# Ajay-Wong/seq2seq-attention-asr

Measured on AMD Instinct MI355X. Metric: log-mel frames/sec fwd+bwd, Chorowski TIMIT baseline, higher is better.
Workload: dtype fp32; 1 GPU; BASELINE config 2: timit_chorowski_b32; model=timit/model_chorowski_baseline.lua, global_batch=32, utterances_per_gpu=32, seq_len=128, label_len=40, feat_dim=123, parallelism=dp1, allreduce=none, launch=hipGraph replay

## Files before the change

### seq2seq-attention-asr_amd/csrc/gru_persist.hip

```cpp
#include <algorithm>
#include <cstdlib>

#include "decisions.h"
#include "gru.h"
#include "gru_persist.h"
#include "handoff.h"
#include "skinny.h"

namespace s2s {

namespace {

struct PDir {
  const float* xp;
  long ldxp;
  const float* Wa;
  const float* Wb;
  float* y;
  long ldy;
  float* sv;
  const float* dy;
  long lddy;
  float* dA;
  long ldA;
// ... 79 lines not shown
  float* part;
  unsigned* ticket;
  unsigned long long* stamps;
};

struct PArgs {
  XProj xq;
  int fused;
  PDir d[2];
  int B, L, H, MT, nwg;
  int nmem, nchains;
  int allow_local;
  unsigned* abort_word;
  unsigned* census;
  const int* len;
  char* next_sync;
  size_t next_prep;
  GruPackJobs pack;
  int ring;
  int stream_sweep;
  unsigned long long* stamps;
  unsigned long long* pstamps;
  int prefetch, prefetch_wg;
  unsigned* progress;
  WArgs wg;
};

#ifndef S2S_GRU_DIAG
#define S2S_GRU_DIAG 0
#endif
constexpr int kStampSlots = S2S_GRU_DIAG ? 16 : 8;
#define GRU_STAMP(ph)                                                                      \
  do {                                                                                     \
    if (a.stamps && threadIdx.x == 0)                                                      \
      a.stamps[((long)lw * a.L + s) * kStampSlots + (ph)] = __builtin_amdgcn_s_memrealtime(); \
  } while (0)
#define GRU_STAMP_V(ph, v)                                                                 \
  do {                                                                                     \
    if (a.stamps && threadIdx.x == 0) a.stamps[((long)lw * a.L + s) * kStampSlots + (ph)] = (v); \
  } while (0)
#if S2S_GRU_DIAG
template <int NC>
__device__ __forceinline__ bool sweep_sent_n(float4 (&a)[NC], __amdgpu_buffer_rsrc_t rs, long tbase, int rowt,
                                             int wave, int lane, unsigned* abort_word, unsigned& n) {
  const long lo = tbase + 4 * tile_lane(rowt, lane);
  unsigned spins = 0;
  while (true) {
    ++n;
    bool ok = true;
#pragma unroll
    for (int i = 0; i < NC; ++i) {
      const long off = lo + 4L * 256 * (wave + 4 * i);
      const uint4 p = __builtin_bit_cast(uint4, __builtin_amdgcn_raw_buffer_load_b128(rs, (int)off, 0, 16));
      ok = ok && p.x != kSent && p.y != kSent && p.z != kSent && p.w != kSent;
      a[i] = make_float4(__uint_as_float(p.x), __uint_as_float(p.y), __uint_as_float(p.z), __uint_as_float(p.w));
    }
    if (__all(ok)) return true;
    if (spin_give_up(spins, abort_word)) return false;
  }
}
#define SWEEP_SENT(slot_, ...) sweep_sent_n<NC>(__VA_ARGS__, npoll[slot_])
#else
#define SWEEP_SENT(slot_, ...) sweep_sent_tile<NC>(__VA_ARGS__)
#endif
std::atomic<unsigned long long*> g_gru_stamps[2] = {{nullptr}, {nullptr}};
std::atomic<unsigned long long*> g_gru_pstamps[2] = {{nullptr}, {nullptr}};
std::atomic<unsigned long long*> g_gru_wstamps{nullptr};
constexpr int kProdStampItems = 32;

__device__ __forceinline__ float reduce_or_abort(SkinnyRed& red, int* abort_lds, bool ok, floatx4 acc, int wave,
                                                 int lane, int tid, bool* aborted) {
  if (!ok) *abort_lds = 1;
  const float s = skinny_reduce(red, acc, wave, lane, tid);
  *aborted = *abort_lds != 0;
  return s;
}

template <bool NN, int D>
__device__ __forceinline__ void xproj_produce(const PArgs& a, float* lds, int p, int nprod) {
  const XProj& q = a.xq;
  const int tid = threadIdx.x, lane = tid & 63, wave = tid >> 6;
  const int nk = q.K / 32;
  __shared__ int last_part;
  const int nd = q.nd;
  if (tid >= 256) {
    XUnit x;
    for (int it = 0; xunit_of(q, nd, p, nprod, it, x); ++it) {
      const int nb = 1 + nk / x.P + (q.alpha ? 1 : 0);
      for (int i = 0; i < nb; ++i) __syncthreads();
      if (x.P == 1) {
        __syncthreads();
      } else {
        __syncthreads();
        __syncthreads();
        if (last_part) __syncthreads();
      }
    }
    return;
  }
  const int wy = wave >> 1, wx = wave & 1, li = lane & 31, lk = lane >> 5;
  const int B = a.B, L = a.L, H3 = q.ncd;
  constexpr int LDK = 36;
  float* As[2] = {lds, lds + 64 * LDK};
  float* Bs[2] = {lds + 128 * LDK, lds + 192 * LDK};
  int item = 0;
  XUnit xu;
  for (; xunit_of(q, nd, p, nprod, item, xu); ++item) {
    if (a.pstamps && tid == 0 && item < kProdStampItems)
      a.pstamps[((long)p * kProdStampItems + item) * 2] = __builtin_amdgcn_s_memrealtime();
// ... 210 lines not shown
    const int upto = nr ? ready + (int)__builtin_ctzll(nr) : ready + 64;
    if (upto <= need && spin_give_up(spins, abort_word)) break;
    ready = upto;
  }
}

__device__ __forceinline__ void prep_next_sync(const PArgs& a, int sp, int nsp) {
  if (!a.next_sync) return;
  if (sp == 0 && threadIdx.x == 0) {
    unsigned* hdr = reinterpret_cast<unsigned*>(a.next_sync);
    const unsigned e = __hip_atomic_fetch_add(&g_s2s_epoch_ctr, 1u, __ATOMIC_RELAXED, __HIP_MEMORY_SCOPE_AGENT) + 1u;
    __hip_atomic_exchange(hdr + kEpochWord, e, __ATOMIC_RELAXED, __HIP_MEMORY_SCOPE_AGENT);
    rearm_abort_word(hdr);
  }
  const size_t n16 = (a.next_prep - 256) / 16;
  uint4* p = reinterpret_cast<uint4*>(a.next_sync + 256);
  for (size_t i = (size_t)sp * blockDim.x + threadIdx.x; i < n16; i += (size_t)nsp * blockDim.x)
    p[i] = make_uint4(0u, 0u, 0u, 0u);
  if (threadIdx.x == 0 && sp == 0 && (a.next_prep - 256) % 16) {
    unsigned* t = reinterpret_cast<unsigned*>(a.next_sync + 256 + n16 * 16);
    for (size_t i = 0; i < ((a.next_prep - 256) % 16) / 4; ++i) t[i] = 0u;
  }
}

constexpr int kRowRing = 4;
constexpr int kSentRing = 4;
__device__ __forceinline__ int sent_slot(const PArgs& a, int s) { return a.ring ? (s & (a.ring - 1)) : s; }
__device__ __forceinline__ void rearm_tile(float* role, const PArgs& a, int s, long tile, int lane) {
  const float4 sv = make_float4(__uint_as_float(kSent), __uint_as_float(kSent), __uint_as_float(kSent),
                                __uint_as_float(kSent));
  *reinterpret_cast<float4*>(role + (long)sent_slot(a, s) * a.MT * 16 * a.H + tile + 4 * lane) = sv;
}
constexpr int kFwdThreads = 320;
template <int NC>
__global__ __launch_bounds__(kFwdThreads) void gru_fwd_persist(PArgs a) {
  __shared__ SkinnyRed red;
  __shared__ int abort_lds, local_lds;
  __shared__ unsigned tb_lds;
  __shared__ __attribute__((aligned(16))) float hprev[16][16];
  __shared__ __attribute__((aligned(16))) float xring[kRowRing][2][256];
  __shared__ __attribute__((aligned(16))) float stg[2][3][256];
  extern __shared__ __attribute__((aligned(16))) float xlds[];
  const int H = a.H, B = a.B, L = a.L;
  const ChainSlot cs = chain_slot(a.nmem);
  if (cs.chain >= a.nchains) {
    const int gch = 8 * ((a.nchains + 7) / 8);
    const int sp = (cs.chain - a.nchains) * a.nmem + cs.member, nsp = (gch - a.nchains) * a.nmem;
    prep_next_sync(a, sp, nsp);
    if (a.fused) xproj_produce_any<false>(a, xlds, sp, nsp);
    for (int j = 0; j < a.pack.n; ++j)
      gru_pack_elems(a.pack.j[j], (long)sp * blockDim.x + threadIdx.x, (long)nsp * blockDim.x);
    return;
  }
  const int dir = cs.chain / a.MT, mt = cs.chain % a.MT;
  const PDir& g = a.d[dir];
  const int ncol = 2 * H / 16;
  const int c1 = cs.member;
  const int lw = dir * a.nwg + mt * ncol + c1;
  const bool isz = c1 < H / 16;
  const int tid = threadIdx.x, lane = tid & 63, wave = tid >> 6;
  const int b0 = mt * 16;
  if (tid == 0) abort_lds = 0;
  const unsigned tb = launch_tagbase(a.abort_word, &tb_lds);
  const bool loader = wave == 4;
  const long mytile = (long)mt * 16 * H + (long)(isz ? c1 : c1 - H / 16) * 256;
  if (!loader)
    rearm_rect((isz ? g.s0 : g.s1) + mytile, (long)a.MT * 16 * H, a.ring ? a.ring : L, 16, 0, 16, 0, 16);
// ... 59 lines not shown
      if (s > 0) store(s - 1);
      put(s + 2, ra);
      issue(s + 3, ra);
      if (ring) {
        if (isz && s >= 2) rearm_tile(g.s0, a, s - 2, mytile, lane);
        if (!isz && s >= 1) rearm_tile(g.s1, a, s - 1, mytile, lane);
      }
      if (!isz) continue;
      __syncthreads();
      if (abort_lds) return;
    }
    __syncthreads();
    store(L - 1);
    return;
  }

  float4 w1[NC], w2[NC];
  load_wfrag(w1, g.Wa + (long)(c1 * 16 + (lane & 15)) * H, wave, lane);
  if (isz) load_wfrag(w2, g.Wb + (long)(c1 * 16 + (lane & 15)) * H, wave, lane);

  const __amdgpu_buffer_rsrc_t hg = rsrc_of(g.g0), qg = rsrc_of(g.g1), hs = rsrc_of(g.s0), qs = rsrc_of(g.s1);
  const long slot = (long)B * H;
  const long slotS = (long)a.MT * 16 * H, tileS = (long)mt * 16 * H;
  const int rowt = min(b0 + (lane & 15), B - 1) - b0;
  const int br = min(b0 + (lane & 15), B - 1);
  const int ob = b0 + (tid >> 4), on = c1 * 16 + (tid & 15);
  const bool live = ob < B;
  const int lenb = (a.len && live) ? a.len[ob] : L;
  const int jt = c1 * 16 - H, wt = (jt % 64) / 16, it = jt / 64;
  float zreg = 0.f, hreg = 0.f;
  bool aborted = false;

  __syncthreads();
  for (int s = 0; s < L; ++s) {
    const int t = g.reverse ? L - 1 - s : s;
    floatx4 acc = {0.f, 0.f, 0.f, 0.f};
    bool ok = true;
    GRU_STAMP(0);
    if (s > 0) {
      float4 av[NC];
#if S2S_GRU_DIAG
      unsigned npoll[1] = {0};
#endif
      {
      if (loc) ok = SWEEP_SENT(0, av, hs, 4 * (sent_slot(a, s - 1) * slotS + tileS), rowt, wave, lane, a.abort_word);
      else ok = sweep_skinny<NC>(av, hg, 8 * (((s - 1) & 1) * slot + (long)br * H), tb + s, wave, lane, a.abort_word);
      GRU_STAMP(1);
#if S2S_GRU_DIAG
      GRU_STAMP_V(8, npoll[0]);
#endif
      acc = mfma_chunks<NC>(av, w1);
      }
      if (!isz && wave == wt) {
#pragma unroll
        for (int i = 0; i < NC; ++i)
          if (i == it) *reinterpret_cast<float4*>(&hprev[lane & 15][4 * (lane >> 4)]) = av[i];
      }
    }
    GRU_STAMP(6);
    float sum = reduce_or_abort(red, &abort_lds, ok, acc, wave, lane, tid, &aborted);
    GRU_STAMP(7);
    const float xpv = xring[s % kRowRing][0][tid], xph = xring[s % kRowRing][1][tid];
    const float hpark = hprev[tid >> 4][tid & 15];
    {
      const float gate = gru_sigmoid(sum + xpv);
      float* st3 = &stg[s & 1][0][tid];
      if (isz) {
        st3[0] = gate;
        zreg = gate;
      } else {
        const int j = on - H;
        const float hp = s > 0 ? hpark : 0.f;
        const float q = gate * hp;
        if (loc) {
          if (live) put_sent(g.s1 + sent_slot(a, s) * slotS + tile_off(ob, j, H), q);
        } else {
          put_granule_pair(g.g1, (s & 1) * slot + (long)ob * H + j, q, tb + s + 1, live);
        }
        st3[0] = gate;
        st3[256] = hp;
        st3[512] = q;
      }
    }
    GRU_STAMP(2);
    if (aborted) return;
    if (!isz) continue;
    acc = floatx4{0.f, 0.f, 0.f, 0.f};
    ok = true;
    GRU_STAMP(3);
    if (s > 0) {
      float4 av[NC];
#if S2S_GRU_DIAG
      unsigned npoll[1] = {0};
#endif
      {
      if (loc) ok = SWEEP_SENT(0, av, qs, 4 * (sent_slot(a, s) * slotS + tileS), rowt, wave, lane, a.abort_word);
      else ok = sweep_skinny<NC>(av, qg, 8 * ((s & 1) * slot + (long)br * H), tb + s + 1, wave, lane, a.abort_word);
      GRU_STAMP(4);
#if S2S_GRU_DIAG
      GRU_STAMP_V(9, npoll[0]);
#endif
      acc = mfma_chunks<NC>(av, w2);
      }
    }
    sum = reduce_or_abort(red, &abort_lds, ok, acc, wave, lane, tid, &aborted);
    {
      const float hh = gru_tanh(sum + xph);
      const float hp = hreg;
      hreg = (-zreg + 1.0f) * hp + zreg * hh;
      if (t >= lenb) hreg = 0.f;
      if (loc) {
        if (live) put_sent(g.s0 + sent_slot(a, s) * slotS + tile_off(ob, on, H), hreg);
      } else {
        put_granule_pair(g.g0, (s & 1) * slot + (long)ob * H + on, hreg, tb + s + 1, live);
      }
      stg[s & 1][1][tid] = hh;
      stg[s & 1][2][tid] = hreg;
    }
    GRU_STAMP(5);
    if (aborted) return;
  }
  __syncthreads();
}

constexpr int kBwdThreads = 320;

template <int NC>
__device__ __forceinline__ void bptt_prefetch(const PArgs& a, int chain, int w, int nwg) {
  if (threadIdx.x >= 256) return;
  const int tid = threadIdx.x, L = a.L, H = a.H, B = a.B, nmem = a.nmem;
  const int tasks = 64 * nmem / nwg, task0 = w * tasks;
  const int dir = chain / a.MT, mt = chain % a.MT;
  const PDir& g = a.d[dir];
  const unsigned* prog = a.progress + (long)chain * nmem;
  int yready = 0, have = 0;
  float sink = 0.f;
  __shared__ int have_lds[2];
  int it = 0;
  constexpr int kMaxTasks = NC;
  for (int q = 3; q < L; ++q, ++it) {
    if (tid == 0) {
      unsigned spins = 0;
      bool gave_up = false;
      while (have + 3 + a.prefetch < q) {
        have = (int)__hip_atomic_load(prog, __ATOMIC_RELAXED, __HIP_MEMORY_SCOPE_AGENT);
        if (have + 3 + a.prefetch >= q) break;
        if (spin_give_up(spins, a.abort_word)) {
          gave_up = true;
          break;
        }
      }
      have_lds[it & 1] = gave_up ? -1 : have;
    }
    __syncthreads();
    const int hv = have_lds[it & 1];
    if (hv < 0) return;
    have = hv;
    if (q < have + 4) q = have + 4;
// ... 177 lines not shown
  const __amdgpu_buffer_rsrc_t pr = rsrc_of(q.part);
  const int tile = 3 * H * NP;
  const int mine = (dir * a.MT + mt) * tile + row0 * NP + (4 * kq) * NP + cb0 * 16 + jl;
#pragma unroll
  for (int c = 0; c < kWgCB; ++c) {
    if (cb0 + c >= nblk) continue;
#pragma unroll
    for (int r = 0; r < 4; ++r)
#pragma unroll
      for (int e = 0; e < 4; ++e)
        __builtin_amdgcn_raw_buffer_store_b32(__float_as_uint(acc[r][c][e]), pr, 4 * (mine + (16 * r + e) * NP + 16 * c),
                                              0, 16);
  }
  asm volatile("s_waitcnt vmcnt(0)" ::: "memory");
  __syncthreads();
  if (tid == 0)
    *flag_lds = (int)__hip_atomic_fetch_add(q.ticket + dir * q.nw + w, 1u, __ATOMIC_RELAXED, __HIP_MEMORY_SCOPE_AGENT);
  __syncthreads();
  if (*flag_lds != a.MT - 1) return;
  const long ldw = (long)H + D;
  float* dW = q.dW[dir][gate];
  const int u0 = row0 - gate * H, first = dir * a.MT * tile + row0 * NP;
  for (int idx = tid; idx < 64 * NP; idx += 256) {
    const int rr = idx / NP, j = idx - rr * NP;
    if (j >= H + D) continue;
    float sum = __uint_as_float(__builtin_amdgcn_raw_buffer_load_b32(pr, 4 * (first + idx), 0, 16));
    for (int m = 1; m < a.MT; ++m)
      sum += __uint_as_float(__builtin_amdgcn_raw_buffer_load_b32(pr, 4 * (first + m * tile + idx), 0, 16));
    float* o = dW + (long)(u0 + rr) * ldw + j;
    *o = q.scale * sum + *o;
  }
}

template <int NC>
__global__ __launch_bounds__(kBwdThreads) void gru_bwd_persist(PArgs a) {
  __shared__ SkinnyRed red;
  __shared__ int abort_lds, local_lds;
  __shared__ unsigned tb_lds;
  __shared__ __attribute__((aligned(16))) float rowq[kRowRing][5][256];
  extern __shared__ __attribute__((aligned(16))) float ylds[];
  const int H = a.H, B = a.B, L = a.L;
  const ChainSlot cs = chain_slot(a.nmem);
  const int gch = 8 * ((a.nchains + 7) / 8);
  if ((int)blockIdx.x >= chain_grid(a.nchains, a.nmem)) {
    const int pre = chain_grid(a.nchains, a.nmem) + (a.prefetch ? 8 * a.prefetch_wg : 0);
    if ((int)blockIdx.x < pre) {
      const int e = (int)blockIdx.x - chain_grid(a.nchains, a.nmem), c = e & 7, w = e >> 3;
      if (c < a.nchains) bptt_prefetch<NC>(a, c, w, a.prefetch_wg);
      return;
    }
    const int e = (int)blockIdx.x - pre, c = e & 7, w = e >> 3;
    if (c < a.nchains) bptt_wgrad<NC>(a, c, w, &tb_lds, &abort_lds);
    return;
  }
  if (cs.chain >= a.nchains) {
    const int sp = (cs.chain - a.nchains) * a.nmem + cs.member, nsp = (gch - a.nchains) * a.nmem;
    prep_next_sync(a, sp, nsp);
    if (a.fused) xproj_produce_any<true>(a, ylds, sp, nsp);
    return;
  }
  const int dir = cs.chain / a.MT, mt = cs.chain % a.MT;
  const PDir& g = a.d[dir];
  const int ncol = H / 16;
  const int c = cs.member;
  const int lw = dir * a.nwg + mt * ncol + c;
  const int tid = threadIdx.x, lane = tid & 63, wave = tid >> 6;
  const int b0 = mt * 16;
  if (a.stamps && tid == 0) a.stamps[((long)lw * L + L - 1) * 8 + 6] = __builtin_amdgcn_s_memrealtime();
  if (tid == 0) abort_lds = 0;
  const unsigned tb = launch_tagbase(a.abort_word, &tb_lds);
  const bool loader = wave == 4;
  const long mytile = (long)mt * 16 * H + (long)c * 256;
  if (!loader) {
    const long st = (long)a.MT * 16 * H;
    const int ns = a.ring ? a.ring : L;
    rearm_rect(g.s0 + mytile, st, ns, 16, 0, 16, 0, 16);
    rearm_rect(g.s1 + mytile, st, ns, 16, 0, 16, 0, 16);
    rearm_rect(g.s2 + mytile, st, ns, 16, 0, 16, 0, 16);
  }
  rearm_done();
  const bool loc = chain_is_local(a.census, cs.chain, a.nmem, c, a.allow_local != 0, a.abort_word, &local_lds, tb);
  if (a.stamps && tid == 0) a.stamps[((long)lw * L + L - 1) * 8 + 7] = __builtin_amdgcn_s_memrealtime();

  if (loader) {
    const int bl = b0 + (lane >> 2), u = c * 16 + 4 * (lane & 3);
    const bool lv = bl < B;
    const int lenl = (a.len && lv) ? a.len[bl] : L;
    const __amdgpu_buffer_rsrc_t dyr = rsrc_of(g.dy);
    int yready = 0;
    auto issue = [&](int q, float4 (&r)[5]) {
#pragma unroll
      for (int v = 0; v < 5; ++v) r[v] = make_float4(0.f, 0.f, 0.f, 0.f);
      if (q >= L) return;
      if (a.fused) xproj_wait(a.xq, dir, q / a.xq.tpt, yready, lane, a.abort_word);
      if (!lv) return;
#ifdef S2S_EXP_NOLOAD
      return;
#endif
      const int t = g.reverse ? q : L - 1 - q;
      const long row = (long)bl * L + t;
      const float* sv = g.sv + row * 5 * H + u;
#pragma unroll
      for (int v = 0; v < 4; ++v) r[v] = *reinterpret_cast<const float4*>(sv + v * H);
      if (t >= lenl) return;
      if (a.fused) {
        r[4] = __builtin_bit_cast(float4, __builtin_amdgcn_raw_buffer_load_b128(
                                              dyr, (int)(4 * (row * g.lddy + u)), 0, 16));
      } else {
        r[4] = *reinterpret_cast<const float4*>(g.dy + row * g.lddy + u);
      }
    };
    auto put = [&](int q, const float4 (&r)[5]) {
#pragma unroll
      for (int v = 0; v < 5; ++v) *reinterpret_cast<float4*>(&rowq[q % kRowRing][v][4 * lane]) = r[v];
    };
    float4 ra[5], rb[5];
    issue(0, ra);
    issue(1, rb);
    put(0, ra);
    put(1, rb);
    issue(2, ra);
    __syncthreads();
    const bool ring = a.ring && loc;
    unsigned* prog = a.progress ? a.progress + (long)cs.chain * a.nmem + c : nullptr;
    for (int p = 0; p < L; ++p) {
      __syncthreads();
      if (abort_lds) return;
      put(p + 2, ra);
      if (prog && lane == 0) __hip_atomic_store(prog, (unsigned)p, __ATOMIC_RELAXED, __HIP_MEMORY_SCOPE_WORKGROUP);
#ifndef S2S_EXP_LOADB
      issue(p + 3, ra);
#endif
      if (ring && p >= 1) {
        rearm_tile(g.s0, a, p - 1, mytile, lane);
        rearm_tile(g.s1, a, p - 1, mytile, lane);
        rearm_tile(g.s2, a, p - 1, mytile, lane);
      }
      asm volatile("s_waitcnt vmcnt(0)" ::: "memory");
      __syncthreads();
      if (abort_lds) return;
#ifdef S2S_EXP_LOADB
      issue(p + 3, ra);
#endif
    }
    if (a.wg.nw) {
      __syncthreads();
      if (lane == 0) __hip_atomic_store(prog, (unsigned)L + 3u, __ATOMIC_RELAXED, __HIP_MEMORY_SCOPE_AGENT);
    }
    return;
  }

  float4 wh[NC], wzr[2 * NC];
  load_wfrag(wh, g.Wa + (long)(c * 16 + (lane & 15)) * H, wave, lane);
  load_wfrag(wzr, g.Wb + (long)(c * 16 + (lane & 15)) * 2 * H, wave, lane);
  const __amdgpu_buffer_rsrc_t zg = rsrc_of(g.g0), rg = rsrc_of(g.g1), hg = rsrc_of(g.g2);
  const __amdgpu_buffer_rsrc_t zs = rsrc_of(g.s0), rs_ = rsrc_of(g.s1), hs = rsrc_of(g.s2);
  const long slot = (long)B * H;
  const int br = min(b0 + (lane & 15), B - 1);
  const long slotS = (long)a.MT * 16 * H, tileS = (long)mt * 16 * H;
  const int rowt = br - b0;
  const int ob = b0 + (tid >> 4), ok_ = c * 16 + (tid & 15);
  const bool live = ob < B;
  const int lenb = (a.len && live) ? a.len[ob] : L;
  float dhc = 0.f, dhp = 0.f;
  bool aborted = false;

  struct Row {
    float z, r, hh, hp, dy;
  };
  auto load_row = [&](int q) {
    const float(*r)[256] = rowq[q % kRowRing];
    return Row{r[0][tid], r[1][tid], r[2][tid], r[3][tid], r[4][tid]};
  };
  auto gate = [&](int t, const Row& v, float dh, int pn, bool pub) {
    const long row = (long)ob * L + t;
    const float daz = dh * (v.hh - v.hp) * (v.z * (1.0f - v.z));
    const float dah = (dh * v.z) * (1.0f - v.hh * v.hh);
    if (loc) {
      const long off = sent_slot(a, pn) * slotS + tile_off(ob, ok_, H);
      if (pub) {
        put_sent(g.s2 + off, dah);
        put_sent(g.s0 + off, daz);
      }
    } else {
      const long off = (pn & 1) * slot + (long)ob * H + ok_;
      put_granule_pair(g.g2, off, dah, tb + pn + 1, pub);
      put_granule_pair(g.g0, off, daz, tb + pn + 1, pub);
    }
#ifndef S2S_EXP_NODA
    if (pub) {
      g.dA[row * g.ldA + ok_] = daz;
      g.dA[row * g.ldA + 2 * H + ok_] = dah;
    }
#endif
  };

  const int tl = g.reverse ? 0 : L - 1;
  __syncthreads();
  Row cur = load_row(0);
  gate(tl, cur, cur.dy, 0, live);

  for (int p = 0; p < L; ++p) {
    const int s = L - 1 - p;
    const int t = g.reverse ? L - 1 - s : s;
    const long row = (long)ob * L + t;
    const unsigned tag = tb + p + 1;
    const int sl = p & 1;
    float4 av[NC];
    GRU_STAMP(0);
#if S2S_GRU_DIAG
    unsigned npoll[3] = {0, 0, 0};
#endif
    bool ok;
    floatx4 acc;
    uint4 zraw[NC];
    bool zpre = false;
#if !S2S_GRU_DIAG
    if (loc && a.stream_sweep) {
      floatx4 acc0 = {0.f, 0.f, 0.f, 0.f}, acc1 = {0.f, 0.f, 0.f, 0.f};
      ok = sweep_sent_mfma<NC>(av, hs, 4 * (sent_slot(a, p) * slotS + tileS), rowt, wave, lane, wh, acc0, acc1,
                               a.abort_word);
      GRU_STAMP(1);
      if constexpr (NC % 2 == 0) {
        sent_tile_issue<NC>(zraw, zs, 4 * (sent_slot(a, p) * slotS + tileS), rowt, wave, lane);
        zpre = true;
      }
      acc = acc0 + acc1;
    } else
#endif
    {
    ok = loc ? SWEEP_SENT(0, av, hs, 4 * (sent_slot(a, p) * slotS + tileS), rowt, wave, lane, a.abort_word)
             : sweep_skinny<NC>(av, hg, 8 * (sl * slot + (long)br * H), tag, wave, lane, a.abort_word);
    GRU_STAMP(1);
#if S2S_GRU_DIAG
    GRU_STAMP_V(8, npoll[0]);
#endif
    acc = mfma_chunks<NC>(av, wh);
    }
    const float dq = reduce_or_abort(red, &abort_lds, ok, acc, wave, lane, tid, &aborted);
    if (loc) {
      if (live) put_sent(g.s1 + sent_slot(a, p) * slotS + tile_off(ob, ok_, H), (dq * cur.hp) * (cur.r * (1.0f - cur.r)));
    } else {
      put_granule_pair(g.g1, sl * slot + (long)ob * H + ok_, (dq * cur.hp) * (cur.r * (1.0f - cur.r)), tag, live);
    }
    if (live) {
      const float dar = (dq * cur.hp) * (cur.r * (1.0f - cur.r));
#ifndef S2S_EXP_NODA
      g.dA[row * g.ldA + H + ok_] = dar;
#endif
      const float dh = cur.dy + dhc;
      dhp = dh * (-cur.z + 1.0f) + dq * cur.r;
    }
    GRU_STAMP(2);
    if (aborted) return;
    const int tn = g.reverse ? t + 1 : t - 1;
    float4 azr[2 * NC];
    GRU_STAMP(3);
    bool split = false;
    if constexpr (NC % 2 == 0 && !S2S_GRU_DIAG) split = loc;
    if constexpr (NC % 2 == 0 && !S2S_GRU_DIAG) if (split) {
      float4 az[NC], ar[NC];
      uint4 rraw[NC];
      ok = true;
      if (!zpre || !sent_tile_check<NC>(zraw, az))
        ok = sweep_sent_tile<NC>(az, zs, 4 * (sent_slot(a, p) * slotS + tileS), rowt, wave, lane, a.abort_word);
      sent_tile_issue<NC>(rraw, rs_, 4 * (sent_slot(a, p) * slotS + tileS), rowt, wave, lane);
      floatx4 acc0 = {0.f, 0.f, 0.f, 0.f}, acc1 = {0.f, 0.f, 0.f, 0.f};
      __builtin_amdgcn_sched_barrier(0);
      mfma_pairs<NC>(az, wzr, acc0, acc1);
      __builtin_amdgcn_sched_barrier(0);
      if (!sent_tile_check<NC>(rraw, ar))
        ok = ok && sweep_sent_tile<NC>(ar, rs_, 4 * (sent_slot(a, p) * slotS + tileS), rowt, wave, lane, a.abort_word);
      GRU_STAMP(4);
      mfma_pairs<NC>(ar, wzr + NC, acc0, acc1);
      acc = acc0 + acc1;
    }
    if (!split) {
      float4 az[NC], ar[NC];
      if (loc) {
        ok = SWEEP_SENT(1, az, zs, 4 * (sent_slot(a, p) * slotS + tileS), rowt, wave, lane, a.abort_word);
#if S2S_GRU_DIAG
        GRU_STAMP(10);
#endif
        ok = ok && SWEEP_SENT(2, ar, rs_, 4 * (sent_slot(a, p) * slotS + tileS), rowt, wave, lane, a.abort_word);
#if S2S_GRU_DIAG
        GRU_STAMP_V(9, npoll[1]);
        GRU_STAMP_V(11, npoll[2]);
#endif
      } else {
        ok = sweep_skinny<NC>(az, zg, 8 * (sl * slot + (long)br * H), tag, wave, lane, a.abort_word);
        ok = ok && sweep_skinny<NC>(ar, rg, 8 * (sl * slot + (long)br * H), tag, wave, lane, a.abort_word);
      }
      GRU_STAMP(4);
#pragma unroll
      for (int i = 0; i < NC; ++i) { azr[i] = az[i]; azr[NC + i] = ar[i]; }
      acc = mfma_chunks<2 * NC>(azr, wzr);
    }
    const float sm = reduce_or_abort(red, &abort_lds, ok, acc, wave, lane, tid, &aborted);
    const Row nxt = s > 0 ? load_row(p + 1) : Row{0.f, 0.f, 0.f, 0.f, 0.f};
    if (live && s > 0) dhc = tn < lenb ? dhp + sm : 0.f;
    if (s > 0) gate(tn, nxt, nxt.dy + dhc, p + 1, live);
    cur = nxt;
    GRU_STAMP(5);
    if (aborted) return;
  }
  if (a.wg.nw) {
    asm volatile("s_waitcnt vmcnt(0)" ::: "memory");
    __syncthreads();
  }
}

constexpr int kExclLds = 124 * 1024;

std::atomic<int> g_bptt_prefetch_wg{2};
std::atomic<int> g_bptt_prefetch{8};
int bptt_prefetch_wg(int ndir, int B, int H) {
  const int nch = ndir * ((B + 15) / 16), nm = H / 16;
  const int nwg = std::max(1, std::min((int)g_bptt_prefetch_wg, nm));
  return g_bptt_prefetch > 0 && nch <= 8 && nm + nwg <= 32 && nm % nwg == 0 ? nwg : 0;
}
std::atomic<int> g_allow_local{1};
std::atomic<int> g_sent_ring{kSentRing};
std::atomic<int> g_stream_sweep{1};

template <int NC>
int launch_nc(hipStream_t st, const PArgs& a, bool excl_req, bool fwd) {
  const dim3 grid(chain_grid(a.nchains, a.nmem) + (!fwd && a.prefetch ? 8 * a.prefetch_wg : 0) +
                  (!fwd ? 8 * a.wg.nw : 0));
  const bool excl = excl_req && a.nchains <= 8 && a.nmem <= 32;
  const unsigned shm = excl ? kExclLds : (a.fused ? kXpLds : 0);
  if (fwd) {
    if (excl) S2S_CHECK_HIP(hipFuncSetAttribute(reinterpret_cast<const void*>(gru_fwd_persist<NC>),
                                                hipFuncAttributeMaxDynamicSharedMemorySize, kExclLds));
    S2S_TRY(check_resident(reinterpret_cast<const void*>(gru_fwd_persist<NC>), grid.x, kFwdThreads, shm,
                           "gru_fwd_persist"));
    hipLaunchKernelGGL(gru_fwd_persist<NC>, grid, dim3(kFwdThreads), shm, st, a);
  } else {
    if (excl) S2S_CHECK_HIP(hipFuncSetAttribute(reinterpret_cast<const void*>(gru_bwd_persist<NC>),
                                                hipFuncAttributeMaxDynamicSharedMemorySize, kExclLds));
    S2S_TRY(check_resident(reinterpret_cast<const void*>(gru_bwd_persist<NC>), grid.x, kBwdThreads, shm,
                           "gru_bwd_persist"));
    hipLaunchKernelGGL(gru_bwd_persist<NC>, grid, dim3(kBwdThreads), shm, st, a);
  }
  S2S_CHECK_HIP(hipGetLastError());
  return 0;
}

int launch(hipStream_t st, const PArgs& a, bool excl, bool fwd) {
  switch (a.H / 64) {
    case 1: return launch_nc<1>(st, a, excl, fwd);
    case 2: return launch_nc<2>(st, a, excl, fwd);
    case 4: return launch_nc<4>(st, a, excl, fwd);
    case 8: return launch_nc<8>(st, a, excl, fwd);
  }
  set_error("gru persistent: unsupported H");
  return 2;
}

}

std::atomic<int> g_fuse_xproj{1};

bool gru_persist_fused_xproj(int ndir, int B, int H, int Kx) {
  if (!g_fuse_xproj || B > 64 || Kx % 32 != 0 || H % 64 != 0) return false;
  const int MT = (B + 15) / 16, nchains = ndir * MT, nmem = 2 * H / 16;
  return chain_grid(nchains, nmem) - nchains * nmem >= 32;
}

std::atomic<int> g_xp_split{1};
std::atomic<int> g_fuse_dy{1};

bool gru_persist_fused_dy(int ndir, int B, int H, int K, long ldw, long lddy) {
  if (!g_fuse_xproj || !g_fuse_dy || B > 64 || K % 32 != 0 || H % 64 != 0 || ldw % 4 != 0 || lddy < (long)ndir * H) return false;
  const int MT = (B + 15) / 16, nchains = ndir * MT, nmem = H / 16;
  return chain_grid(nchains, nmem) - nchains * nmem >= 32;
}

bool gru_persist_wgrad_fits(int ndir, int B, int H, int D) {
  const int nch = ndir * ((B + 15) / 16), nm = H / 16, nw = 3 * H / 64;
  return H % 64 == 0 && D > 0 && nch <= 8 && nm + bptt_prefetch_wg(ndir, B, H) + nw <= 32 &&
         H + (D + 15) / 16 * 16 <= 4 * kWgCB * 16;
}

bool gru_persist_supported(int ndir, int B, int H) {
  if (!(H == 64 || H == 128 || H == 256 || H == 512)) return false;
  const int MT = (B + 15) / 16;
// ... 300 lines not shown
    o[2 * i] = r;
    o[2 * i + 1] = c;
    while (__builtin_amdgcn_s_memrealtime() - r < period) __builtin_amdgcn_s_sleep(2);
  }
}
int clock_probe_launch(hipStream_t st, int nwg, int n, int period, unsigned long long* out) {
  S2S_REQUIRE(nwg > 0 && nwg <= 64 && n > 0 && n <= (1 << 20) && period > 0 && (double)n * period < 2e8,
              "clock probe: bad arguments");
  hipLaunchKernelGGL(clock_probe_kernel, dim3(nwg), dim3(64), 0, st, out, n, (unsigned long long)period);
  S2S_CHECK_HIP(hipGetLastError());
  return 0;
}

}

extern "C" int s2s_debug_clock_probe(void* stream, int nwg, int n, int period, unsigned long long* out) {
  return s2s::clock_probe_launch(static_cast<hipStream_t>(stream), nwg, n, period, out);
}

extern "C" int s2s_debug_lds_hog(void* stream, int nwg, int lds_bytes, double usec, float* out) {
  return s2s::lds_hog_launch(static_cast<hipStream_t>(stream), nwg, lds_bytes, usec, out);
}

extern "C" void s2s_debug_gru_local(int allow) { s2s::g_allow_local = allow; }
extern "C" void s2s_debug_gru_fused_xproj(int on) { s2s::g_fuse_xproj = on; }
extern "C" void s2s_debug_gru_fused_dy(int on) { s2s::g_fuse_dy = on; }
extern "C" void s2s_debug_gru_xp_split(int on) { s2s::g_xp_split = on; }
extern "C" void s2s_debug_gru_xp_group(int on) { s2s::g_xp_group = on; }
extern "C" void s2s_debug_bptt_prefetch(int wg, int lookahead) {
  s2s::g_bptt_prefetch_wg = wg;
  s2s::g_bptt_prefetch = lookahead;
}
extern "C" void s2s_debug_gru_stream_sweep(int on) { s2s::g_stream_sweep = on; }
extern "C" void s2s_debug_gru_ring(int on) { s2s::g_sent_ring = on ? s2s::kSentRing : 0; }
extern "C" void s2s_debug_gru_stamps(void* fwd, void* bwd) {
  s2s::g_gru_stamps[0] = static_cast<unsigned long long*>(fwd);
  s2s::g_gru_stamps[1] = static_cast<unsigned long long*>(bwd);
}
extern "C" void s2s_debug_gru_wg_stamps(void* p) { s2s::g_gru_wstamps = static_cast<unsigned long long*>(p); }
extern "C" void s2s_debug_gru_prod_stamps(void* fwd, void* bwd) {
  s2s::g_gru_pstamps[0] = static_cast<unsigned long long*>(fwd);
  s2s::g_gru_pstamps[1] = static_cast<unsigned long long*>(bwd);
}
```

Before: 1.393 million frames/s.

## Add lean specialized GRU persistent kernels with strength-reduced sentinel addressing

```diff
diff --git a/seq2seq-attention-asr_amd/csrc/gru_persist.hip b/seq2seq-attention-asr_amd/csrc/gru_persist.hip
--- a/seq2seq-attention-asr_amd/csrc/gru_persist.hip
+++ b/seq2seq-attention-asr_amd/csrc/gru_persist.hip
@@ -135,12 +135,14 @@
 constexpr int kStampSlots = S2S_GRU_DIAG ? 16 : 8;
 #define GRU_STAMP(ph)                                                                      \
   do {                                                                                     \
-    if (a.stamps && threadIdx.x == 0)                                                      \
-      a.stamps[((long)lw * a.L + s) * kStampSlots + (ph)] = __builtin_amdgcn_s_memrealtime(); \
+    if constexpr (DIAG)                                                                    \
+      if (a.stamps && threadIdx.x == 0)                                                    \
+        a.stamps[((long)lw * a.L + s) * kStampSlots + (ph)] = __builtin_amdgcn_s_memrealtime(); \
   } while (0)
 #define GRU_STAMP_V(ph, v)                                                                 \
   do {                                                                                     \
-    if (a.stamps && threadIdx.x == 0) a.stamps[((long)lw * a.L + s) * kStampSlots + (ph)] = (v); \
+    if constexpr (DIAG)                                                                    \
+      if (a.stamps && threadIdx.x == 0) a.stamps[((long)lw * a.L + s) * kStampSlots + (ph)] = (v); \
   } while (0)
 #if S2S_GRU_DIAG
 template <int NC>
@@ -178,6 +180,35 @@
   *aborted = *abort_lds != 0;
   return s;
 }
+
+template <class T>
+__device__ __forceinline__ T keep_v(T x) {
+  asm volatile("" : "+v"(x));
+  return x;
+}
+template <class T>
+__device__ __forceinline__ T* keep_g(T* p) {
+  unsigned long v = reinterpret_cast<unsigned long>(p);
+  asm volatile("" : "+v"(v));
+  return (T*)(__attribute__((address_space(1))) T*)v;
+}
+template <class T>
+__device__ __forceinline__ T* keep_sg(T* p) {
+  const unsigned long u = reinterpret_cast<unsigned long>(p);
+  unsigned long v = ((unsigned long)(unsigned)__builtin_amdgcn_readfirstlane((int)(u >> 32)) << 32) |
+                    (unsigned)__builtin_amdgcn_readfirstlane((int)u);
+  asm volatile("" : "+s"(v));
+  return (T*)(__attribute__((address_space(1))) T*)v;
+}
+__device__ __forceinline__ int keep_s(int x) {
+  x = __builtin_amdgcn_readfirstlane(x);
+  asm volatile("" : "+s"(x));
+  return x;
+}
+template <bool B>
+struct BoolC {
+  static constexpr bool value = B;
+};
 
 template <bool NN, int D>
 __device__ __forceinline__ void xproj_produce(const PArgs& a, float* lds, int p, int nprod) {
@@ -454,7 +485,7 @@
   *reinterpret_cast<float4*>(role + (long)sent_slot(a, s) * a.MT * 16 * a.H + tile + 4 * lane) = sv;
 }
 constexpr int kFwdThreads = 320;
-template <int NC>
+template <int NC, bool LEAN, bool DIAG>
 __global__ __launch_bounds__(kFwdThreads) void gru_fwd_persist(PArgs a) {
   __shared__ SkinnyRed red;
   __shared__ int abort_lds, local_lds;
@@ -580,8 +611,36 @@
   bool aborted = false;
 
   __syncthreads();
-  for (int s = 0; s < L; ++s) {
-    const int t = g.reverse ? L - 1 - s : s;
+  auto recur = [&](auto lr) -> bool {
+  constexpr bool LR = decltype(lr)::value;
+  const bool loc_o = loc, isz_o = isz, live_o = live;
+  const bool loc = LR || loc_o;
+  const bool isz = LR ? keep_s(isz_o) != 0 : isz_o;
+  const bool live = LR ? keep_v((int)live_o) != 0 : live_o;
+  const int Ls = LR ? keep_s(L) : L, wtk = LR ? keep_s(wt) : wt, itk = LR ? keep_s(it) : it;
+  unsigned* const abw = LR ? keep_sg(a.abort_word) : a.abort_word;
+  float* pub = nullptr;
+  int slotSb = 0, tileSb = 0, so_cur = 0, so_prev = 0, tv = 0, dtv = 0, lenk = lenb, rowk = rowt;
+  if constexpr (LR) {
+    pub = keep_g((isz_o ? g.s0 + tile_off(ob, on, H) : g.s1 + tile_off(ob, on - H, H)));
+    slotSb = keep_v((int)(4 * slotS));
+    tileSb = keep_v((int)(4 * tileS));
+    tv = keep_v(g.reverse ? L - 1 : 0);
+    dtv = keep_v(g.reverse ? -1 : 1);
+    lenk = keep_v(lenb);
+    rowk = keep_v(rowt);
+  }
+  auto advance = [&](int s) {
+    if constexpr (LR) {
+      so_prev = so_cur;
+      so_cur = ((s + 1) & (kSentRing - 1)) ? so_cur + slotSb : 0;
+      tv += dtv;
+    }
+  };
+  for (int s = 0; s < Ls; advance(s), ++s) {
+    const int t = LR ? tv : (g.reverse ? L - 1 - s : s);
+    const long sw_prev = LR ? (long)(tileSb + so_prev) : 4 * (sent_slot(a, s - 1) * slotS + tileS);
+    const long sw_cur = LR ? (long)(tileSb + so_cur) : 4 * (sent_slot(a, s) * slotS + tileS);
     floatx4 acc = {0.f, 0.f, 0.f, 0.f};
     bool ok = true;
     GRU_STAMP(0);
@@ -591,18 +650,18 @@
       unsigned npoll[1] = {0};
 #endif
       {
-      if (loc) ok = SWEEP_SENT(0, av, hs, 4 * (sent_slot(a, s - 1) * slotS + tileS), rowt, wave, lane, a.abort_word);
-      else ok = sweep_skinny<NC>(av, hg, 8 * (((s - 1) & 1) * slot + (long)br * H), tb + s, wave, lane, a.abort_word);
+      if (loc) ok = SWEEP_SENT(0, av, hs, sw_prev, rowk, wave, lane, abw);
+      else ok = sweep_skinny<NC>(av, hg, 8 * (((s - 1) & 1) * slot + (long)br * H), tb + s, wave, lane, abw);
       GRU_STAMP(1);
 #if S2S_GRU_DIAG
       GRU_STAMP_V(8, npoll[0]);
 #endif
       acc = mfma_chunks<NC>(av, w1);
       }
-      if (!isz && wave == wt) {
+      if (!isz && wave == wtk) {
 #pragma unroll
         for (int i = 0; i < NC; ++i)
-          if (i == it) *reinterpret_cast<float4*>(&hprev[lane & 15][4 * (lane >> 4)]) = av[i];
+          if (i == itk) *reinterpret_cast<float4*>(&hprev[lane & 15][4 * (lane >> 4)]) = av[i];
       }
     }
     GRU_STAMP(6);
@@ -621,7 +680,11 @@
         const float hp = s > 0 ? hpark : 0.f;
         const float q = gate * hp;
         if (loc) {
-          if (live) put_sent(g.s1 + sent_slot(a, s) * slotS + tile_off(ob, j, H), q);
+          if constexpr (LR) {
+            if (live) put_sent(reinterpret_cast<float*>(reinterpret_cast<char*>(pub) + so_cur), q);
+          } else {
+            if (live) put_sent(g.s1 + sent_slot(a, s) * slotS + tile_off(ob, j, H), q);
+          }
         } else {
           put_granule_pair(g.g1, (s & 1) * slot + (long)ob * H + j, q, tb + s + 1, live);
         }
@@ -631,7 +694,7 @@
       }
     }
     GRU_STAMP(2);
-    if (aborted) return;
+    if (aborted) return true;
     if (!isz) continue;
     acc = floatx4{0.f, 0.f, 0.f, 0.f};
     ok = true;
@@ -642,8 +705,8 @@
       unsigned npoll[1] = {0};
 #endif
       {
-      if (loc) ok = SWEEP_SENT(0, av, qs, 4 * (sent_slot(a, s) * slotS + tileS), rowt, wave, lane, a.abort_word);
-      else ok = sweep_skinny<NC>(av, qg, 8 * ((s & 1) * slot + (long)br * H), tb + s + 1, wave, lane, a.abort_word);
+      if (loc) ok = SWEEP_SENT(0, av, qs, sw_cur, rowk, wave, lane, abw);
+      else ok = sweep_skinny<NC>(av, qg, 8 * ((s & 1) * slot + (long)br * H), tb + s + 1, wave, lane, abw);
       GRU_STAMP(4);
 #if S2S_GRU_DIAG
       GRU_STAMP_V(9, npoll[0]);
@@ -656,9 +719,13 @@
       const float hh = gru_tanh(sum + xph);
       const float hp = hreg;
       hreg = (-zreg + 1.0f) * hp + zreg * hh;
-      if (t >= lenb) hreg = 0.f;
+      if (t >= lenk) hreg = 0.f;
       if (loc) {
-        if (live) put_sent(g.s0 + sent_slot(a, s) * slotS + tile_off(ob, on, H), hreg);
+        if constexpr (LR) {
+          if (live) put_sent(reinterpret_cast<float*>(reinterpret_cast<char*>(pub) + so_cur), hreg);
+        } else {
+          if (live) put_sent(g.s0 + sent_slot(a, s) * slotS + tile_off(ob, on, H), hreg);
+        }
       } else {
         put_granule_pair(g.g0, (s & 1) * slot + (long)ob * H + on, hreg, tb + s + 1, live);
       }
@@ -666,12 +733,21 @@
       stg[s & 1][2][tid] = hreg;
     }
     GRU_STAMP(5);
-    if (aborted) return;
-  }
+    if (aborted) return true;
+  }
+  return false;
+  };
+  bool gone;
+  if constexpr (LEAN) gone = (loc && a.ring == kSentRing) ? recur(BoolC<true>{}) : recur(BoolC<false>{});
+  else gone = recur(BoolC<false>{});
+  if (gone) return;
   __syncthreads();
 }
 
 constexpr int kBwdThreads = 320;
+#ifndef S2S_EXP_BWD_LEAN
+#define S2S_EXP_BWD_LEAN 2
+#endif
 
 template <int NC>
 __device__ __forceinline__ void bptt_prefetch(const PArgs& a, int chain, int w, int nwg) {
@@ -915,7 +991,7 @@
   }
 }
 
-template <int NC>
+template <int NC, bool LEAN, bool DIAG>
 __global__ __launch_bounds__(kBwdThreads) void gru_bwd_persist(PArgs a) {
   __shared__ SkinnyRed red;
   __shared__ int abort_lds, local_lds;
@@ -932,8 +1008,10 @@
       if (c < a.nchains) bptt_prefetch<NC>(a, c, w, a.prefetch_wg);
       return;
     }
-    const int e = (int)blockIdx.x - pre, c = e & 7, w = e >> 3;
-    if (c < a.nchains) bptt_wgrad<NC>(a, c, w, &tb_lds, &abort_lds);
+    if constexpr (!LEAN) {
+      const int e = (int)blockIdx.x - pre, c = e & 7, w = e >> 3;
+      if (c < a.nchains) bptt_wgrad<NC>(a, c, w, &tb_lds, &abort_lds);
+    }
     return;
   }
   if (cs.chain >= a.nchains) {
@@ -949,7 +1027,8 @@
   const int lw = dir * a.nwg + mt * ncol + c;
   const int tid = threadIdx.x, lane = tid & 63, wave = tid >> 6;
   const int b0 = mt * 16;
-  if (a.stamps && tid == 0) a.stamps[((long)lw * L + L - 1) * 8 + 6] = __builtin_amdgcn_s_memrealtime();
+  if constexpr (DIAG)
+    if (a.stamps && tid == 0) a.stamps[((long)lw * L + L - 1) * 8 + 6] = __builtin_amdgcn_s_memrealtime();
   if (tid == 0) abort_lds = 0;
   const unsigned tb = launch_tagbase(a.abort_word, &tb_lds);
   const bool loader = wave == 4;
@@ -963,7 +1042,8 @@
   }
   rearm_done();
   const bool loc = chain_is_local(a.census, cs.chain, a.nmem, c, a.allow_local != 0, a.abort_word, &local_lds, tb);
-  if (a.stamps && tid == 0) a.stamps[((long)lw * L + L - 1) * 8 + 7] = __builtin_amdgcn_s_memrealtime();
+  if constexpr (DIAG)
+    if (a.stamps && tid == 0) a.stamps[((long)lw * L + L - 1) * 8 + 7] = __builtin_amdgcn_s_memrealtime();
 
   if (loader) {
     const int bl = b0 + (lane >> 2), u = c * 16 + 4 * (lane & 3);
@@ -1026,7 +1106,7 @@
       issue(p + 3, ra);
 #endif
     }
-    if (a.wg.nw) {
+    if (!LEAN && a.wg.nw) {
       __syncthreads();
       if (lane == 0) __hip_atomic_store(prog, (unsigned)L + 3u, __ATOMIC_RELAXED, __HIP_MEMORY_SCOPE_AGENT);
     }
@@ -1055,11 +1135,48 @@
     const float(*r)[256] = rowq[q % kRowRing];
     return Row{r[0][tid], r[1][tid], r[2][tid], r[3][tid], r[4][tid]};
   };
-  auto gate = [&](int t, const Row& v, float dh, int pn, bool pub) {
+  auto recur = [&](auto lr) -> bool {
+  constexpr bool LR = decltype(lr)::value;
+  constexpr int HC = 64 * NC;
+  const bool loc_o = loc, live_o = live;
+  const bool loc = LR || loc_o;
+  const bool live = LR ? keep_v((int)live_o) != 0 : live_o;
+  const int Ls = LR ? keep_s(L) : L;
+  unsigned* const abw = LR ? keep_sg(a.abort_word) : a.abort_word;
+  char *pubz = nullptr, *pubr = nullptr, *pubh = nullptr, *dAcur = nullptr;
+  long dAstep = 0;
+  int slotSb = 0, tileSb = 0, so_cur = 0, so_next = 0, tv = 0, dtv = 0, lenk = lenb, rowk = rowt;
+  if constexpr (LR) {
+    const long to = tile_off(ob, ok_, H);
+    const int t0 = g.reverse ? 0 : L - 1, dt = g.reverse ? 1 : -1;
+    pubz = keep_g(reinterpret_cast<char*>(g.s0 + to));
+    pubr = keep_g(reinterpret_cast<char*>(g.s1 + to));
+    pubh = keep_g(reinterpret_cast<char*>(g.s2 + to));
+    dAcur = keep_g(reinterpret_cast<char*>(g.dA + ((long)ob * L + t0) * g.ldA + ok_));
+    dAstep = keep_v(4 * g.ldA * dt);
+    slotSb = keep_v((int)(4 * slotS));
+    tileSb = keep_v((int)(4 * tileS));
+    so_next = slotSb;
+    tv = keep_v(t0);
+    dtv = keep_v(dt);
+    lenk = keep_v(lenb);
+    rowk = keep_v(rowt);
+  }
+  auto gate = [&](int t, const Row& v, float dh, int pn, bool pub, int so, char* dArow) {
     const long row = (long)ob * L + t;
     const float daz = dh * (v.hh - v.hp) * (v.z * (1.0f - v.z));
     const float dah = (dh * v.z) * (1.0f - v.hh * v.hh);
-    if (loc) {
+    if constexpr (LR) {
+      if (pub) {
+        put_sent(reinterpret_cast<float*>(pubh + so), dah);
+        put_sent(reinterpret_cast<float*>(pubz + so), daz);
+#ifndef S2S_EXP_NODA
+        reinterpret_cast<float*>(dArow)[0] = daz;
+        reinterpret_cast<float*>(dArow)[2 * HC] = dah;
+#endif
+      }
+      return;
+    } else if (loc) {
       const long off = sent_slot(a, pn) * slotS + tile_off(ob, ok_, H);
       if (pub) {
         put_sent(g.s2 + off, dah);
@@ -1079,16 +1196,16 @@
   };
 
   const int tl = g.reverse ? 0 : L - 1;
-  __syncthreads();
   Row cur = load_row(0);
-  gate(tl, cur, cur.dy, 0, live);
-
-  for (int p = 0; p < L; ++p) {
-    const int s = L - 1 - p;
-    const int t = g.reverse ? L - 1 - s : s;
+  gate(tl, cur, cur.dy, 0, live, 0, dAcur);
+
+  for (int p = 0; p < Ls; ++p) {
+    const int s = Ls - 1 - p;
+    const int t = LR ? tv : (g.reverse ? L - 1 - s : s);
     const long row = (long)ob * L + t;
     const unsigned tag = tb + p + 1;
     const int sl = p & 1;
+    const long sw_cur = LR ? (long)(tileSb + so_cur) : 4 * (sent_slot(a, p) * slotS + tileS);
     float4 av[NC];
     GRU_STAMP(0);
 #if S2S_GRU_DIAG
@@ -1099,21 +1216,20 @@
     uint4 zraw[NC];
     bool zpre = false;
 #if !S2S_GRU_DIAG
-    if (loc && a.stream_sweep) {
+    if (LR || (loc && a.stream_sweep)) {
       floatx4 acc0 = {0.f, 0.f, 0.f, 0.f}, acc1 = {0.f, 0.f, 0.f, 0.f};
-      ok = sweep_sent_mfma<NC>(av, hs, 4 * (sent_slot(a, p) * slotS + tileS), rowt, wave, lane, wh, acc0, acc1,
-                               a.abort_word);
+      ok = sweep_sent_mfma<NC>(av, hs, sw_cur, rowk, wave, lane, wh, acc0, acc1, abw);
       GRU_STAMP(1);
       if constexpr (NC % 2 == 0) {
-        sent_tile_issue<NC>(zraw, zs, 4 * (sent_slot(a, p) * slotS + tileS), rowt, wave, lane);
+        sent_tile_issue<NC>(zraw, zs, sw_cur, rowk, wave, lane);
         zpre = true;
       }
       acc = acc0 + acc1;
     } else
 #endif
     {
-    ok = loc ? SWEEP_SENT(0, av, hs, 4 * (sent_slot(a, p) * slotS + tileS), rowt, wave, lane, a.abort_word)
-             : sweep_skinny<NC>(av, hg, 8 * (sl * slot + (long)br * H), tag, wave, lane, a.abort_word);
+    ok = loc ? SWEEP_SENT(0, av, hs, sw_cur, rowk, wave, lane, abw)
+             : sweep_skinny<NC>(av, hg, 8 * (sl * slot + (long)br * H), tag, wave, lane, abw);
     GRU_STAMP(1);
 #if S2S_GRU_DIAG
     GRU_STAMP_V(8, npoll[0]);
@@ -1121,7 +1237,9 @@
     acc = mfma_chunks<NC>(av, wh);
     }
     const float dq = reduce_or_abort(red, &abort_lds, ok, acc, wave, lane, tid, &aborted);
-    if (loc) {
+    if constexpr (LR) {
+      if (live) put_sent(reinterpret_cast<float*>(pubr + so_cur), (dq * cur.hp) * (cur.r * (1.0f - cur.r)));
+    } else if (loc) {
       if (live) put_sent(g.s1 + sent_slot(a, p) * slotS + tile_off(ob, ok_, H), (dq * cur.hp) * (cur.r * (1.0f - cur.r)));
     } else {
       put_granule_pair(g.g1, sl * slot + (long)ob * H + ok_, (dq * cur.hp) * (cur.r * (1.0f - cur.r)), tag, live);
@@ -1129,14 +1247,15 @@
     if (live) {
       const float dar = (dq * cur.hp) * (cur.r * (1.0f - cur.r));
 #ifndef S2S_EXP_NODA
-      g.dA[row * g.ldA + H + ok_] = dar;
+      if constexpr (LR) reinterpret_cast<float*>(dAcur)[HC] = dar;
+      else g.dA[row * g.ldA + H + ok_] = dar;
 #endif
       const float dh = cur.dy + dhc;
       dhp = dh * (-cur.z + 1.0f) + dq * cur.r;
     }
     GRU_STAMP(2);
-    if (aborted) return;
-    const int tn = g.reverse ? t + 1 : t - 1;
+    if (aborted) return true;
+    const int tn = LR ? tv + dtv : (g.reverse ? t + 1 : t - 1);
     float4 azr[2 * NC];
     GRU_STAMP(3);
     bool split = false;
@@ -1146,14 +1265,14 @@
       uint4 rraw[NC];
       ok = true;
       if (!zpre || !sent_tile_check<NC>(zraw, az))
-        ok = sweep_sent_tile<NC>(az, zs, 4 * (sent_slot(a, p) * slotS + tileS), rowt, wave, lane, a.abort_word);
-      sent_tile_issue<NC>(rraw, rs_, 4 * (sent_slot(a, p) * slotS + tileS), rowt, wave, lane);
+        ok = sweep_sent_tile<NC>(az, zs, sw_cur, rowk, wave, lane, abw);
+      sent_tile_issue<NC>(rraw, rs_, sw_cur, rowk, wave, lane);
       floatx4 acc0 = {0.f, 0.f, 0.f, 0.f}, acc1 = {0.f, 0.f, 0.f, 0.f};
       __builtin_amdgcn_sched_barrier(0);
       mfma_pairs<NC>(az, wzr, acc0, acc1);
       __builtin_amdgcn_sched_barrier(0);
       if (!sent_tile_check<NC>(rraw, ar))
-        ok = ok && sweep_sent_tile<NC>(ar, rs_, 4 * (sent_slot(a, p) * slotS + tileS), rowt, wave, lane, a.abort_word);
+        ok = ok && sweep_sent_tile<NC>(ar, rs_, sw_cur, rowk, wave, lane, abw);
       GRU_STAMP(4);
       mfma_pairs<NC>(ar, wzr + NC, acc0, acc1);
       acc = acc0 + acc1;
@@ -1161,18 +1280,18 @@
     if (!split) {
       float4 az[NC], ar[NC];
       if (loc) {
-        ok = SWEEP_SENT(1, az, zs, 4 * (sent_slot(a, p) * slotS + tileS), rowt, wave, lane, a.abort_word);
+        ok = SWEEP_SENT(1, az, zs, sw_cur, rowk, wave, lane, abw);
 #if S2S_GRU_DIAG
         GRU_STAMP(10);
 #endif
-        ok = ok && SWEEP_SENT(2, ar, rs_, 4 * (sent_slot(a, p) * slotS + tileS), rowt, wave, lane, a.abort_word);
+        ok = ok && SWEEP_SENT(2, ar, rs_, sw_cur, rowk, wave, lane, abw);
 #if S2S_GRU_DIAG
         GRU_STAMP_V(9, npoll[1]);
         GRU_STAMP_V(11, npoll[2]);
 #endif
       } else {
-        ok = sweep_skinny<NC>(az, zg, 8 * (sl * slot + (long)br * H), tag, wave, lane, a.abort_word);
-        ok = ok && sweep_skinny<NC>(ar, rg, 8 * (sl * slot + (long)br * H), tag, wave, lane, a.abort_word);
+        ok = sweep_skinny<NC>(az, zg, 8 * (sl * slot + (long)br * H), tag, wave, lane, abw);
+        ok = ok && sweep_skinny<NC>(ar, rg, 8 * (sl * slot + (long)br * H), tag, wave, lane, abw);
       }
       GRU_STAMP(4);
 #pragma unroll
@@ -1181,13 +1300,28 @@
     }
     const float sm = reduce_or_abort(red, &abort_lds, ok, acc, wave, lane, tid, &aborted);
     const Row nxt = s > 0 ? load_row(p + 1) : Row{0.f, 0.f, 0.f, 0.f, 0.f};
-    if (live && s > 0) dhc = tn < lenb ? dhp + sm : 0.f;
-    if (s > 0) gate(tn, nxt, nxt.dy + dhc, p + 1, live);
+    if (live && s > 0) dhc = tn < lenk ? dhp + sm : 0.f;
+    if (s > 0) gate(tn, nxt, nxt.dy + dhc, p + 1, live, so_next, dAcur + dAstep);
     cur = nxt;
     GRU_STAMP(5);
-    if (aborted) return;
-  }
-  if (a.wg.nw) {
+    if (aborted) return true;
+    if constexpr (LR) {
+      so_cur = so_next;
+      so_next = ((p + 2) & (kSentRing - 1)) ? so_next + slotSb : 0;
+      tv += dtv;
+      dAcur += dAstep;
+    }
+  }
+  return false;
+  };
+  __syncthreads();
+  bool gone;
+  if constexpr (LEAN && S2S_EXP_BWD_LEAN == 2)
+    gone = (loc && a.ring == kSentRing && a.stream_sweep) ? recur(BoolC<true>{}) : recur(BoolC<false>{});
+  else
+    gone = recur(BoolC<false>{});
+  if (gone) return;
+  if (!LEAN && a.wg.nw) {
     asm volatile("s_waitcnt vmcnt(0)" ::: "memory");
     __syncthreads();
   }
@@ -1206,35 +1340,46 @@
 std::atomic<int> g_sent_ring{kSentRing};
 std::atomic<int> g_stream_sweep{1};
 
-template <int NC>
+std::atomic<int> g_gru_lean{1};
+
+template <int NC, bool LEAN, bool DIAG>
 int launch_nc(hipStream_t st, const PArgs& a, bool excl_req, bool fwd) {
   const dim3 grid(chain_grid(a.nchains, a.nmem) + (!fwd && a.prefetch ? 8 * a.prefetch_wg : 0) +
                   (!fwd ? 8 * a.wg.nw : 0));
   const bool excl = excl_req && a.nchains <= 8 && a.nmem <= 32;
   const unsigned shm = excl ? kExclLds : (a.fused ? kXpLds : 0);
   if (fwd) {
-    if (excl) S2S_CHECK_HIP(hipFuncSetAttribute(reinterpret_cast<const void*>(gru_fwd_persist<NC>),
+    const auto kern = gru_fwd_persist<NC, LEAN, DIAG>;
+    if (excl) S2S_CHECK_HIP(hipFuncSetAttribute(reinterpret_cast<const void*>(kern),
                                                 hipFuncAttributeMaxDynamicSharedMemorySize, kExclLds));
-    S2S_TRY(check_resident(reinterpret_cast<const void*>(gru_fwd_persist<NC>), grid.x, kFwdThreads, shm,
-                           "gru_fwd_persist"));
-    hipLaunchKernelGGL(gru_fwd_persist<NC>, grid, dim3(kFwdThreads), shm, st, a);
+    S2S_TRY(check_resident(reinterpret_cast<const void*>(kern), grid.x, kFwdThreads, shm, "gru_fwd_persist"));
+    hipLaunchKernelGGL(kern, grid, dim3(kFwdThreads), shm, st, a);
   } else {
-    if (excl) S2S_CHECK_HIP(hipFuncSetAttribute(reinterpret_cast<const void*>(gru_bwd_persist<NC>),
+    const auto kern = gru_bwd_persist<NC, LEAN, DIAG>;
+    if (excl) S2S_CHECK_HIP(hipFuncSetAttribute(reinterpret_cast<const void*>(kern),
                                                 hipFuncAttributeMaxDynamicSharedMemorySize, kExclLds));
-    S2S_TRY(check_resident(reinterpret_cast<const void*>(gru_bwd_persist<NC>), grid.x, kBwdThreads, shm,
-                           "gru_bwd_persist"));
-    hipLaunchKernelGGL(gru_bwd_persist<NC>, grid, dim3(kBwdThreads), shm, st, a);
+    S2S_TRY(check_resident(reinterpret_cast<const void*>(kern), grid.x, kBwdThreads, shm, "gru_bwd_persist"));
+    hipLaunchKernelGGL(kern, grid, dim3(kBwdThreads), shm, st, a);
   }
   S2S_CHECK_HIP(hipGetLastError());
   return 0;
 }
 
+template <int NC>
+int launch_mode(hipStream_t st, const PArgs& a, bool excl, bool fwd) {
+  const bool lean = g_gru_lean != 0 && a.wg.nw == 0 && (fwd || S2S_EXP_BWD_LEAN != 0);
+  decide("gru.lean", lean);
+  if (!lean) return launch_nc<NC, false, true>(st, a, excl, fwd);
+  if (a.stamps) return launch_nc<NC, true, true>(st, a, excl, fwd);
+  return launch_nc<NC, true, false>(st, a, excl, fwd);
+}
+
 int launch(hipStream_t st, const PArgs& a, bool excl, bool fwd) {
   switch (a.H / 64) {
-    case 1: return launch_nc<1>(st, a, excl, fwd);
-    case 2: return launch_nc<2>(st, a, excl, fwd);
-    case 4: return launch_nc<4>(st, a, excl, fwd);
-    case 8: return launch_nc<8>(st, a, excl, fwd);
+    case 1: return launch_mode<1>(st, a, excl, fwd);
+    case 2: return launch_mode<2>(st, a, excl, fwd);
+    case 4: return launch_mode<4>(st, a, excl, fwd);
+    case 8: return launch_mode<8>(st, a, excl, fwd);
   }
   set_error("gru persistent: unsupported H");
   return 2;
@@ -1601,6 +1746,7 @@
   s2s::g_bptt_prefetch = lookahead;
 }
 extern "C" void s2s_debug_gru_stream_sweep(int on) { s2s::g_stream_sweep = on; }
+extern "C" void s2s_debug_gru_lean(int on) { s2s::g_gru_lean = on; }
 extern "C" void s2s_debug_gru_ring(int on) { s2s::g_sent_ring = on ? s2s::kSentRing : 0; }
 extern "C" void s2s_debug_gru_stamps(void* fwd, void* bwd) {
   s2s::g_gru_stamps[0] = static_cast<unsigned long long*>(fwd);
```

Result: no change. 1.403 million frames/s (median of 6 runs) (+0.7%).
